# cnettel/cnF2freq

Measured on AMD Instinct MI355X. Metric: individual*marker fwd-bwd steps/sec (all 8 shift modes, forward+backward, dosage rows), higher is better.
Workload: dtype f64

## Files before the change

### cnf2freq_amd/csrc/cnf2_kernels.hip

```cpp
#include <hip/hip_runtime.h>

#include <string.h>
#include <type_traits>

#include "cnf2_device.h"
#include "cnf2_lane.h"
#include "cnf2_emtab.h"
#include "cnf2_accum.h"
#include "cnf2_acctab.h"
#include "cnf2_accpath.h"
#include "cnf2_variance.h"

namespace cnf2 {

template <int CTRL>
__device__ __forceinline__ double dpp_mov_all(double v)
{
    int lo = __builtin_amdgcn_mov_dpp(__double2loint(v), CTRL, 0xF, 0xF, true);
    int hi = __builtin_amdgcn_mov_dpp(__double2hiint(v), CTRL, 0xF, 0xF, true);
    return __hiloint2double(hi, lo);
}
template <int K>
__device__ __forceinline__ double swizzle_xor(double v)
{
// ... 884 lines not shown
struct RawSlots {
    uint8_t ap[4];
    double2 su[4];
    double  hw[4];
    double2 tq;
};

template <int TQ_SHIFT>
__device__ __forceinline__ void load_raw_at(const KernelParams& p, const FastCtx& c, int m, int lo_m, int hi_m, RawSlots* r)
{
    m = m < lo_m ? lo_m : (m > hi_m ? hi_m : m);
    const int32_t rows[4] = {c.row_root, c.row_par, c.row_tr, c.row_ot};
#pragma unroll
    for (int k = 0; k < 4; k++) {
        const size_t i = (size_t)rows[k] * p.n_markers + m;
        r->ap[k] = p.allele8[i];
        r->su[k] = p.sure[i];
        r->hw[k] = p.hw[i];
    }
    const int mt = m + TQ_SHIFT;
    r->tq        = p.tq[mt < 0 ? 0 : mt];
}
template <int TQ_SHIFT>
__device__ __forceinline__ void load_raw(const KernelParams& p, const FastCtx& c, int m0, int lo_m, int hi_m, RawSlots* r)
{
    load_raw_at<TQ_SHIFT>(p, c, m0 + c.mi, lo_m, hi_m, r);
}

template <bool CLASSES, bool HOMPAR = false, bool HOMLEAF = false, bool NORESTR = false, bool TIES = false, int STRIDE = TAB_STRIDE,
          int KOFF = 0>
__device__ __forceinline__ void produce_row(const FastCtx& c, double* tab, bool valid, const RawSlots& raw)
{
    if (valid) {
        const Slot root = unpack_slot(raw.ap[0], raw.su[0].x, raw.su[0].y, raw.hw[0]);
        const Slot par  = unpack_slot(raw.ap[1], raw.su[1].x, raw.su[1].y, raw.hw[1]);
        const Slot tr   = unpack_slot(raw.ap[2], raw.su[2].x, raw.su[2].y, raw.hw[2]);
        const Slot ot   = unpack_slot(raw.ap[3], raw.su[3].x, raw.su[3].y, raw.hw[3]);
        double  cw[2];
        double* row = tab + c.mi * STRIDE;
        double* rb = row + c.idx_base;
        emtab_part_to<CLASSES, HOMPAR, HOMLEAF, NORESTR, TIES>(c.pc, root, par, tr, ot,
                               [&](int kind, int e, double v) {
                                   if (KOFF > 0 && kind == 0) return;
                                   const int b  = e & 3;
                                   const int k  = b == 0 ? 0 : (b == 1 ? c.idx_k01 : (b == 2 ? c.idx_k10 : 6));
                                   rb[(kind == 0 ? 0 : (kind == 1 ? TAB_R : TAB_2) + KOFF) + (e >> 2) * 8 + k] = v;
                               },
                               cw);
        if (KOFF > 0) return;
        if ((c.part & 5) == 0) {
            row[TAB_C + c.pc.f * 2 + 0] = cw[0];
            row[TAB_C + c.pc.f * 2 + 1] = cw[1];
        }
        if (c.part == 0) *(double2*)(row + TAB_T) = raw.tq;
    }
}
template <bool CLASSES, bool TIES = false, int STRIDE = TAB_STRIDE, int KOFF = 0>
__device__ __forceinline__ void produce_tile(const KernelParams& p, const FastCtx& c, double* tab, int m0, int last,
                                             const RawSlots& raw, int hom)
{
    if (TIES) {
        produce_row<CLASSES, false, false, false, CLASSES, STRIDE, KOFF>(c, tab, m0 + c.mi <= last, raw);
        return;
    }
    if (hom == 2) produce_row<CLASSES, true, true, false, false, STRIDE>(c, tab, m0 + c.mi <= last, raw);
    else if (hom == 1) produce_row<CLASSES, true, false, false, false, STRIDE>(c, tab, m0 + c.mi <= last, raw);
    else if (hom == 3) produce_row<CLASSES, false, false, true, false, STRIDE>(c, tab, m0 + c.mi <= last, raw);
    else produce_row<CLASSES, false, false, false, false, STRIDE>(c, tab, m0 + c.mi <= last, raw);
}

struct RawRec {
    uint8_t  ap;
    double   s0, s1, hw;
    double   Bp, Cp, Kp, t0, t1, oo;
    uint32_t bits;
    double   tq0, tq1;
};
__device__ __forceinline__ int clamp_marker(int m, int lo_m, int hi_m) { return m < lo_m ? lo_m : (m > hi_m ? hi_m : m); }
__device__ __forceinline__ uint8_t load_root_allele(const KernelParams& p, const FastCtx& c, int m0, int lo_m, int hi_m)
{
    const __attribute__((address_space(1))) uint8_t* a8 = (const __attribute__((address_space(1))) uint8_t*)p.allele8;
    return a8[(size_t)c.row_root * p.n_markers + clamp_marker(m0 + c.mi, lo_m, hi_m)];
}
template <int TQ_SHIFT, bool ONE_MARKER = false>
__device__ __forceinline__ void load_rec(const KernelParams& p, const FastCtx& c, uint32_t rec_row, int m0, int lo_m, int hi_m,
                                         uint8_t ap, RawRec* r)
{
    const int     m = clamp_marker(m0 + c.mi, lo_m, hi_m);
    const size_t  i = (size_t)c.row_root * p.n_markers + m;
    const double2 su = p.sure[i];
    r->ap = ap;
    r->s0 = su.x;
    r->s1 = su.y;
    r->hw = p.hw[i];
    const int v = ((c.pc.P ^ c.pc.f) & 1) ? (ap >> 4) : (ap & 15);
    const double2* q = (const double2*)(p.line_rec + (((size_t)(rec_row + (uint32_t)m) * LINE_VALUES + v) * 2 + c.pc.firstpar));
    const double2 q0 = q[0], q1 = q[1], q2 = q[2];
    r->Bp   = q0.x;
    r->Cp   = q0.y;
    r->Kp   = q1.x;
    r->t0   = q1.y;
    r->t1   = q2.x;
    r->oo   = q2.y;
    r->bits = ((const uint32_t*)q)[12];
    const int mt = m + TQ_SHIFT;
    if (ONE_MARKER) {
        typedef double sd2 __attribute__((ext_vector_type(2)));
        const int mu = __builtin_amdgcn_readfirstlane(mt < 0 ? 0 : mt);
        const sd2 tq = ((const __attribute__((address_space(4))) sd2*)p.tq)[mu];
        r->tq0 = tq.x;
        r->tq1 = tq.y;
    } else {
        const double2 tq = p.tq[mt < 0 ? 0 : mt];
        r->tq0 = tq.x;
        r->tq1 = tq.y;
    }
}
template <bool CLASSES, bool PACKED = false>
__device__ __forceinline__ void produce_row_rec(const FastCtx& c, double* tab, bool valid, const RawRec& raw)
{
    if (valid) {
        const Slot root = unpack_slot(raw.ap, raw.s0, raw.s1, raw.hw);
        LineRec rec;
        rec.Bp   = raw.Bp;
        rec.Cp   = raw.Cp;
        rec.Kp   = raw.Kp;
        rec.t0   = raw.t0;
        rec.t1   = raw.t1;
        rec.oo   = raw.oo;
        rec.bits = raw.bits;
        double  cw[2];
        double* row = tab + c.mi * TAB_STRIDE;
        double* rb  = row + c.idx_base;
        emtab_part_rec<CLASSES, PACKED>(c.pc.P, c.pc.f, root, rec,
                                [&](int kind, int e, double v) {
                                    const int b = e & 3;
                                    const int k = b == 0 ? 0 : (b == 1 ? c.idx_k01 : (b == 2 ? c.idx_k10 : 6));
                                    rb[(kind == 0 ? 0 : (kind == 1 ? TAB_R : TAB_2)) + (e >> 2) * 8 + k] = v;
                                },
                                cw);
        if ((c.part & 5) == 0) {
            row[TAB_C + c.pc.f * 2 + 0] = cw[0];
            row[TAB_C + c.pc.f * 2 + 1] = cw[1];
        }
        if (c.part == 0) *(double2*)(row + TAB_T) = make_double2(raw.tq0, raw.tq1);
    }
}
__global__ __launch_bounds__(256) void line_records_kernel(const LineKey* lines, int n_lines, const uint8_t* allele8,
                                                           const double2* sure, const double* hw, int n_markers, LineRec* out)
{
    const size_t per_line = (size_t)n_markers * LINE_VALUES * 2;
    const size_t t        = (size_t)blockIdx.x * blockDim.x + threadIdx.x;
    if (t >= per_line * (size_t)n_lines) return;
    const int     firstpar = (int)(t & 1), v = (int)((t >> 1) & (LINE_VALUES - 1));
    const size_t  lm = t / (LINE_VALUES * 2);
    const int     m = (int)(lm % (size_t)n_markers);
    const LineKey k = lines[lm / (size_t)n_markers];
    auto slot = [&](int32_t row) {
        const size_t i = (size_t)row * n_markers + m;
        const double2 s = sure[i];
        return unpack_slot(allele8[i], s.x, s.y, hw[i]);
    };
    const Slot par = slot(k.row_par), ga = slot(k.row_a), gb = slot(k.row_b);
    LineRec r;
    line_record_make(k.fl_par, firstpar ? k.fl_b : k.fl_a, firstpar ? k.fl_a : k.fl_b, firstpar, v, par, firstpar ? gb : ga,
                     firstpar ? ga : gb, &r);
    out[t] = r;
}

struct RawOne {
    uint8_t ap;
    double2 su;
    double  hw;
    double2 tq;
};

template <int TQ_SHIFT>
// ... 1269 lines not shown
#pragma unroll
            for (int j = 0; j < NR; j++) S.b[j] *= e[j];
            const bool scale_here = !ODD && (ml & bmask) == 0;
            if (!ODD && __ballot(scale_here)) {
                double bb[NR] = {S.b[0], S.b[1]};
                double bm = S.bmant;
                int    be = S.bexpo;
                bool   bd = S.bdead;
                const double bsum = scale_chain<true>(bb, &bm, &be, &bd);
#pragma unroll
                for (int j = 0; j < NR; j++) S.b[j] = scale_here ? bb[j] : S.b[j];
                S.bmant = scale_here ? bm : S.bmant;
                S.bexpo = scale_here ? be : S.bexpo;
                S.bdead = scale_here ? bd : S.bdead;
                if (any_in_job(__ballot(scale_here && bsum > 0.0 && bsum * CNF2_RESCALE_GUARD < 1.0))) bmask = 1;
            }
            transition_uniform(S.b, r_m.x, r_m.y);
        };
        {
            const int mtop = first + (ntile - 1) * 2;
            load_rec<-1>(pq, cp, rec_row, mtop + moff, first, last, load_root_allele(pq, cp, mtop + moff, first, last), &rraw);
            ap_next = load_root_allele(pq, cp, mtop - 2 + moff, first, last);
        }
        const int    mi2 = lane >> 3, sub = lane & 7;
        for (int t = ntile - 1; t >= 0; t--) {
            const int m0 = first + t * 2;
            produce_row_rec<true, true>(cp, tab, m0 + pmt <= last, rraw);
            load_rec<-1>(pq, cp, rec_row, m0 - 2 + moff, first, last, ap_next, &rraw);
            ap_next = load_root_allele(pq, cp, m0 - 4 + moff, first, last);
            wave_lds_fence();
            if (m0 < last) {
                marker(odd_t(), myrow1, m0 + 1);
                marker(even_t(), myrow0, m0, true);
            } else marker(even_t(), myrow0, m0);
            wave_lds_fence();
            {
                const double* red = tab + mi2 * TS + sub * 8;
                double        d0 = 0.0, d1 = 0.0, d2 = 0.0;
#pragma unroll
                for (int i2 = 0; i2 < 8; i2++) {
                    d0 += red[i2];
                    d1 += red[64 + i2];
                    d2 += red[128 + i2];
                }
                d0 = chain_sum(d0);
                d1 = chain_sum(d1);
                d2 = chain_sum(d2);
                d0 = fmax(d0, 0.0);
                d1 = fmax(d1, 0.0);
                d2 = fmax(d2, 0.0);
                if (sub == 0 && m0 + (mi2 >> 2) <= last) {
                    if (!(p.flags & KP_RAW_DOSAGE)) {
                        const double tsum = d0 + d1 + d2;
                        const double inv  = tsum > 0.0 ? 1.0 / tsum : 0.0;
                        d0 *= inv;
                        d1 *= inv;
                        d2 *= inv;
                    }
                    int ei = eind;
                    asm volatile("" : "+v"(ei));
                    double* out = p.dosage + ((size_t)ei * p.n_markers + (m0 + (mi2 >> 2))) * 3;
                    out[0] = d0;
                    out[1] = d1;
                    out[2] = d2;
                }
            }
            wave_lds_fence();
        }
    }
    if (stamp && fresh_lane() == 0) {
        p.clock_out[0] = __builtin_readcyclecounter() - t_shader;
        p.clock_out[1] = wall_clock64() - t_wall;
    }
}

static_assert(TAB_R == 72 && TAB_2 == 136 && TAB_STRIDE >= 200, "up8_park (cnf2_lane.h) is written for this row layout");
static_assert(TAB_R % 2 == 0 && TAB_2 % 2 == 0 && TAB_STRIDE % 2 == 0, "the A-side runs of a chain (up8_sum_run) are read 16 bytes at a time");
#ifndef CNF2_UP8_ROW_SUMS
#define CNF2_UP8_ROW_SUMS 1
#endif
#ifndef CNF2_UP8_SCALAR_GAP
#define CNF2_UP8_SCALAR_GAP 1
#endif
#ifndef CNF2_UP8_FWD_TILE
#define CNF2_UP8_FWD_TILE 8
#endif
#ifndef CNF2_UP8_FWD_READ
#define CNF2_UP8_FWD_READ 2
#endif
static_assert(CNF2_UP8_FWD_TILE == 1 || (CNF2_UP8_FWD_TILE >= 2 && CNF2_UP8_FWD_TILE % 2 == 0), "a forward tile holds an even number of markers");
static_assert(CNF2_UP8_FWD_TILE == 1 || up8_fwd_buffers(CNF2_UP8_FWD_TILE, 8 * TAB_STRIDE) * CNF2_UP8_FWD_TILE * UP8_FWD_MARKER <= 8 * TAB_STRIDE,
              "the forward tiles live in the wave's eight table rows");
__device__ __forceinline__ void produce_slot_rec(const FastCtx& c, double* slot, const RawRec& raw)
{
    const Slot root = unpack_slot(raw.ap, raw.s0, raw.s1, raw.hw);
    LineRec rec;
    rec.Bp   = raw.Bp;
    rec.Cp   = raw.Cp;
    rec.Kp   = raw.Kp;
    rec.t0   = raw.t0;
    rec.t1   = raw.t1;
    rec.oo   = raw.oo;
    rec.bits = raw.bits;
    double  cw[2];
    double* d = slot + up8_fwd_at(0, c.mi, 0);
    emtab_part_rec<false, true>(c.pc.P, c.pc.f, root, rec,
                                [&](int, int e, double v) {
                                    if (e == 0) d[up8_fwd_at(0, 0, up8_fwd_part(c.part))] = v;
                                },
                                cw);
    if ((c.part & 5) == 0) {
        d[up8_fwd_at(0, 0, up8_fwd_weight(c.pc.f, 0))] = cw[0];
        d[up8_fwd_at(0, 0, up8_fwd_weight(c.pc.f, 1))] = cw[1];
    }
    if (c.part == 0) {
        d[up8_fwd_at(0, 0, up8_fwd_gap(0))] = raw.tq0;
        d[up8_fwd_at(0, 0, up8_fwd_gap(1))] = raw.tq1;
    }
}
struct Up8FwdRow {
    const double*  row;
    const FastCtx& c;
    __device__ __forceinline__ void emission(double (&e)[2], double k) const { emission_from_row(row, c, e, k); }
    __device__ __forceinline__ double2 gap() const { return *(const double2*)(row + TAB_T); }
};
struct Up8FwdSlot {
    double w0, a0, w1, a1, B0[2], B1[2], g0, g1;
    Up8FwdSlot() = default;
    __device__ __forceinline__ Up8FwdSlot(const double* a, const double* w, const double* b)
    {
        constexpr int F = up8_fwd_at(0, 0, 2);
        w0 = w[0];
        a0 = a[0];
        w1 = w[F];
        a1 = a[F];
#pragma unroll
        for (int j = 0; j < 2; j++) {
            B0[j] = b[up8_fwd_at(0, 0, j)];
            B1[j] = b[F + up8_fwd_at(0, 0, j)];
        }
        g0 = b[up8_fwd_at(0, 0, up8_fwd_gap(0) - 4)];
        g1 = b[up8_fwd_at(0, 0, up8_fwd_gap(1) - 4)];
    }
    __device__ __forceinline__ void emission(double (&e)[2], double k) const
    {
        const double cA0 = w0 * a0 * k;
        const double cA1 = w1 * a1 * k;
#pragma unroll
        for (int j = 0; j < 2; j++) e[j] = cA0 * B0[j] + cA1 * B1[j];
    }
    __device__ __forceinline__ double2 gap() const { return make_double2(g0, g1); }
};
__global__ __launch_bounds__(CNF2_BLOCK, CNF2_UNI_MIN_BLOCKS) void fb_unipack8_kernel(KernelParams p)
{
    constexpr int  NR = 2, ROW = UP8_SPILL_ROW, TS = TAB_STRIDE;
    constexpr bool SG = CNF2_UP8_SCALAR_GAP != 0;
    __shared__ __attribute__((aligned(16))) double lds[CNF2_WAVES_PER_BLOCK][8 * TS];

    const int wib   = __builtin_amdgcn_readfirstlane(threadIdx.x >> 6);
    const int wave  = blockIdx.x * CNF2_WAVES_PER_BLOCK + wib;
    const int nwave = gridDim.x * CNF2_WAVES_PER_BLOCK;
    double*   spill = p.spill + (size_t)wave * p.spill_stride;
    const bool stamp = p.clock_out != nullptr && wave == 0;
    unsigned long long t_shader = 0, t_wall = 0;
    if (stamp) {
        t_shader = __builtin_readcyclecounter();
        t_wall   = wall_clock64();
    }

    auto take_job = [&](int strided) {
        if (!p.job_next) return strided;
        int j = 0;
        if (fresh_lane() == 0) j = atomicAdd(p.job_next, 1);
        return __builtin_amdgcn_readfirstlane(j);
    };
    for (int job = take_job(wave); job < p.n_pjobs; job = take_job(job + nwave)) {
        const int        lane = fresh_lane();
        const PackedJob* pj   = p.pjobs + 2 * (size_t)job;
        int           wq   = wib;
        const Window* wins = p.windows;
        KernelParams  pq   = p;
        asm volatile("" : "+s"(wq), "+s"(wins), "+s"(pq.allele8));
        double* const tab = lds[wq];
        const int first = __builtin_amdgcn_readfirstlane(pj[0].first), last = __builtin_amdgcn_readfirstlane(pj[0].last);
        const int chrom = __builtin_amdgcn_readfirstlane(pj[0].chrom);
        FastCtx cp;
        cp.part = lane >> 3;
        cp.mi   = lane & 7;
        const int moff = -cp.mi;
        uint32_t  rec_row;
        {
            const int    pind = pj[cp.mi >> 2].ind[cp.mi & 3];
            const Window wp   = wins[pind];
            make_part(wp, cp.part, &cp.pc, &cp.row_par, &cp.row_tr, &cp.row_ot);
            cp.row_root = wp.row[0];
            rec_row     = (uint32_t)p.line_keys[2 * (size_t)pind + (cp.pc.P ? 1 : 0)] * (uint32_t)p.n_markers;
        }
        cp.idx_base = part_entry_index(cp.part, 0);
        cp.idx_k01  = part_entry_index(cp.part, 1) - cp.idx_base;
        cp.idx_k10  = part_entry_index(cp.part, 2) - cp.idx_base;
        const int rj = up8_job(lane), b0 = up8_b0(lane);
        const int ind = pj[rj >> 2].ind[rj & 3];
// ... 13 lines not shown
        auto any_in_job = [&](unsigned long long ballot) {
            unsigned tl = (unsigned)ballot, th = (unsigned)(ballot >> 32);
            tl |= tl >> 16;
            tl |= tl >> 8;
            th |= th >> 16;
            th |= th >> 8;
            return (((rj & 4) ? th : tl) & jbits) != 0;
        };
        double* const myrow = tab + rj * TS;
        const bool uspill = !(p.flags & KP_NO_DOSAGE);
        const int  uoff   = up8_spill_value(lane);
        const int  ioff   = up8_spill_inv(rj, c.s0);
        const bool vwr    = up8_spill_writer(lane) && uspill;
        const bool iwr    = b0 == 0 && vwr;

        using odd_t  = std::integral_constant<bool, true>;
        using even_t = std::integral_constant<bool, false>;

        double a[NR];
#pragma unroll
        for (int j = 0; j < NR; j++) a[j] = 1.0 / 64.0;
        double mant = 1.0;
        int    expo = 0;
        bool   dead = false;
        double pend = 1.0;
        int    rmask = CNF2_RESCALE_MASK, bmask = CNF2_RESCALE_MASK;
        auto fwd_step = [&](auto odd_tag, const auto& src, int m) {
            constexpr bool ODD = decltype(odd_tag)::value;
            double         e[NR];
            src.emission(e, pend);
            const double2 r  = src.gap();
            const int     ml = m - first;
            double*       sp = spill + (size_t)(ml >> 1) * ROW;
            if (!ODD) {
                double ep[NR];
                src.emission(ep, 1.0);
                const d2v v = {a[0], a[1]};
                const d2v w = {a[0] * ep[0], a[1] * ep[1]};
                if (vwr) {
                    __builtin_nontemporal_store(v, (d2v*)(sp + uoff));
                    __builtin_nontemporal_store(w, (d2v*)(sp + UP8_SPILL_EMIT + uoff));
                }
            }
#pragma unroll
            for (int j = 0; j < NR; j++) a[j] *= e[j];
            pend = 1.0;
            const bool norm_here = m == last || (!ODD && (ml & rmask) == 0);
            if (__ballot(norm_here)) {
                double       mt = mant;
                int          ex = expo;
                bool         dd = dead;
                const double inv = chain_normaliser<true>(a, &mt, &ex, &dd);
                mant = norm_here ? mt : mant;
                expo = norm_here ? ex : expo;
                dead = norm_here ? dd : dead;
                pend = norm_here ? inv : 1.0;
                if (any_in_job(__ballot(norm_here && inv > CNF2_RESCALE_GUARD))) rmask = 1;
                if (iwr && (!ODD || norm_here)) sp[ioff + (ODD ? 1 : 0)] = pend;
            } else if (!ODD) {
                if (iwr) sp[ioff] = 1.0;
            }
            if (m < last) transition_uniform(a, r.x, r.y);
        };
        RawRec  rraw;
        uint8_t ap_next;
        if constexpr (CNF2_UP8_FWD_TILE == 1) {
            const Up8FwdRow src{myrow, c};
            load_rec<0, SG>(pq, cp, rec_row, first + moff, first, last, load_root_allele(pq, cp, first + moff, first, last), &rraw);
            ap_next = load_root_allele(pq, cp, first + 1 + moff, first, last);
            for (int m = first; m <= last; m++) {
                produce_row_rec<false, true>(cp, tab, true, rraw);
                load_rec<0, SG>(pq, cp, rec_row, m + 1 + moff, first, last, ap_next, &rraw);
                ap_next = load_root_allele(pq, cp, m + 2 + moff, first, last);
                wave_lds_fence();
                if ((m - first) & 1) fwd_step(odd_t(), src, m);
                else fwd_step(even_t(), src, m);
                wave_lds_fence();
            }
        } else {
            constexpr int T = CNF2_UP8_FWD_TILE, REGION = 8 * TS;
            const double* const qa = tab + up8_fwd_at(0, rj, up8_fwd_part(b0));
            const double* const qc = tab + up8_fwd_at(0, rj, up8_fwd_weight(0, c.s0));
            const double* const qb = tab + up8_fwd_at(0, rj, up8_fwd_part(4));
            RawRec  rr[2];
            uint8_t ap[2];
            load_rec<0, SG>(pq, cp, rec_row, first + moff, first, last, load_root_allele(pq, cp, first + moff, first, last), &rr[0]);
            load_rec<0, SG>(pq, cp, rec_row, first + 1 + moff, first, last, load_root_allele(pq, cp, first + 1 + moff, first, last), &rr[1]);
            ap[0] = load_root_allele(pq, cp, first + 2 + moff, first, last);
            ap[1] = load_root_allele(pq, cp, first + 3 + moff, first, last);
            int tile = 0;
            for (int m0 = first; m0 <= last; m0 += T, tile++) {
                const int toff = up8_fwd_tile(T, REGION, tile);
#pragma unroll
                for (int t = 0; t < T; t++) {
                    produce_slot_rec(cp, tab + toff + up8_fwd_at(t, 0, 0), rr[t & 1]);
                    load_rec<0, SG>(pq, cp, rec_row, m0 + t + 2 + moff, first, last, ap[t & 1], &rr[t & 1]);
                    ap[t & 1] = load_root_allele(pq, cp, m0 + t + 4 + moff, first, last);
                }
                wave_lds_fence();
                auto slot_at = [&](int t) {
                    const int o = toff + up8_fwd_at(t, 0, 0);
                    return Up8FwdSlot(qa + o, qc + o, qb + o);
                };
                constexpr int RD = CNF2_UP8_FWD_READ < T ? CNF2_UP8_FWD_READ : T;
                static_assert(T % RD == 0, "a forward tile is read in equal parts");
#pragma unroll
                for (int t0 = 0; t0 < T; t0 += RD) {
                    Up8FwdSlot src[RD];
#pragma unroll
                    for (int t = 0; t < RD; t++) src[t] = slot_at(t0 + t);
#pragma unroll
                    for (int t = 0; t < RD; t++) {
                        if (t0 + t == 0 || m0 + t0 + t <= last) {
                            if ((t0 + t) & 1) fwd_step(odd_t(), src[t], m0 + t0 + t);
                            else fwd_step(even_t(), src[t], m0 + t0 + t);
                        }
                    }
                }
                if (up8_fwd_buffers(T, REGION) == 1) wave_lds_fence();
            }
            if (up8_fwd_buffers(T, REGION) == 2) wave_lds_fence();
        }

        const bool   alive  = !dead;
        const double emine  = alive ? (double)expo : -1e300;
        const double emaxd  = fmax(emine, lane_xor8(emine));
        const bool   any_alive = emaxd > -1e299;
        const int    emax   = any_alive ? (int)emaxd : 0;
        int          dsh    = expo - emax;
        dsh                 = dsh < -2000 ? -2000 : dsh;
        const double tmine  = alive ? ldexp(mant, dsh) : 0.0;
        double       T      = tmine + lane_xor8(tmine);
        T += T;
        T += T;
        if (b0 == 0 && c.s2 == 0) {
#pragma unroll
            for (int s1 = 0; s1 < 2; s1++) {
                const int s = c.s0 | (s1 << 1);
#pragma unroll
                for (int s2 = 0; s2 < 2; s2++) {
                    p.factors[je * 8 + (s | (s2 << 2))] = mant;
                    p.fexp[je * 8 + (s | (s2 << 2))]    = alive ? expo : CNF2_LEXP_DEAD;
                }
            }
        }
        if (jlead) {
            p.loglik[je] = any_alive ? T : 8.0;
            p.lexp[je]   = any_alive ? emax : CNF2_LEXP_DEAD;
        }
        if (p.flags & KP_NO_DOSAGE) continue;

        BwdState<NR> S;
#pragma unroll
        for (int j = 0; j < NR; j++) S.b[j] = 1.0;
        S.bmant = 1.0;
        S.bexpo = 0;
        S.bdead = false;
        S.fmant = mant;
        S.fexpo = expo;
        const double xm  = any_alive ? 1.0 / T : 0.0;
        const int    xe  = -emax;
        const bool   chain_on = alive && !(tmine * 2.3538526683701998e17 < T);
        double nx_am[NR], nx_inv_even, nx_inv_odd;
        auto ask_spill = [&](int mn) {
            const double* sp = spill + (size_t)(mn < 0 ? 0 : mn >> 1) * ROW;
            const d2v     v  = __builtin_nontemporal_load((const d2v*)(sp + ((mn & 1) ? UP8_SPILL_EMIT : 0) + uoff));
            nx_am[0]         = v.x;
            nx_am[1]         = v.y;
            const double2 iv = *(const double2*)(sp + ioff);
            nx_inv_even      = iv.x;
            nx_inv_odd       = iv.y;
        };
        auto take_spill = [&]() {
#pragma unroll
            for (int j = 0; j < NR; j++) S.am[j] = nx_am[j];
            S.inv_even = nx_inv_even;
            S.inv_odd  = nx_inv_odd;
        };
        ask_spill(last - first);

        auto marker = [&](auto odd_tag, double* row, int m) {
            constexpr bool ODD = decltype(odd_tag)::value;
// ... 102 lines not shown
                }
                int ei = ind;
                asm volatile("" : "+v"(ei));
                double* out = p.dosage + ((size_t)ei * p.n_markers + m) * 3;
                out[0] = d0;
                out[1] = d1;
                out[2] = d2;
            }
#else
#ifdef CNF2_X_NOPARK
            double x_sum[3];
#endif
#pragma unroll
            for (int h = 0; h < 2; h++) {
                const int s1 = 1 - h;
                double    q[4][3];
#pragma unroll
                for (int v = 0; v < 4; v++) {
                    double n_tot = 0.0, n_a1 = 0.0, n_b1 = 0.0, n_2 = 0.0;
#pragma unroll
                    for (int f = 0; f < 2; f++) {
                        const int    ia = (f << 4) | (s1 << 3) | b0 | (v << 1);
                        const double cf = f ? cf1 : cf0;
                        const double av = cf * row[TAB_R + ia], a1 = cf * row[TAB_2 + ia];
                        const double sb = z[2 * f], sb1 = z[2 * f + 1];
                        n_tot += av * sb;
                        n_a1 += a1 * sb;
                        n_b1 += av * sb1;
                        n_2 += a1 * sb1;
                    }
                    q[v][2] = scale * n_2;
                    q[v][1] = scale * (n_a1 + n_b1 - 2.0 * n_2);
                    q[v][0] = scale * (n_tot - n_a1 - n_b1 + n_2);
#ifdef CNF2_X_NOPARK
#pragma unroll
                    for (int k = 0; k < 3; k++) x_sum[k] = (h == 0 && v == 0 ? 0.0 : x_sum[k]) + q[v][k];
#endif
                }
#ifndef CNF2_X_NOPARK
                wave_lds_fence();
#pragma unroll
                for (int v = 0; v < 4; v++) {
                    const int vl = up8_virtual_lane(lane, s1, v);
                    row[up8_park(0, vl)] = q[v][0];
                    row[up8_park(1, vl)] = q[v][1];
                    row[up8_park(2, vl)] = q[v][2];
                }
#endif
            }
#ifdef CNF2_X_NOPARK
            {
                const double d0 = fmax(chain_sum(x_sum[0]), 0.0), d1 = fmax(chain_sum(x_sum[1]), 0.0), d2 = fmax(chain_sum(x_sum[2]), 0.0);
                const double tsum = d0 + d1 + d2;
                const double inv  = (p.flags & KP_RAW_DOSAGE) ? 1.0 : (tsum > 0.0 ? 1.0 / tsum : 0.0);
                if ((lane & 7) == 0) {
                    int ei = eind;
                    asm volatile("" : "+v"(ei));
                    double* out = p.dosage + ((size_t)ei * p.n_markers + m) * 3;
                    out[0] = d0 * inv;
                    out[1] = d1 * inv;
                    out[2] = d2 * inv;
                }
            }
#endif
#endif
#pragma unroll
            for (int j = 0; j < NR; j++) S.b[j] *= e[j];
            const bool scale_here = !ODD && (ml & bmask) == 0;
            if (!ODD && __ballot(scale_here)) {
                double bb[NR] = {S.b[0], S.b[1]};
                double bm = S.bmant;
                int    be = S.bexpo;
                bool   bd = S.bdead;
                const double bsum = scale_chain<true>(bb, &bm, &be, &bd);
#pragma unroll
                for (int j = 0; j < NR; j++) S.b[j] = scale_here ? bb[j] : S.b[j];
                S.bmant = scale_here ? bm : S.bmant;
                S.bexpo = scale_here ? be : S.bexpo;
                S.bdead = scale_here ? bd : S.bdead;
                if (any_in_job(__ballot(scale_here && bsum > 0.0 && bsum * CNF2_RESCALE_GUARD < 1.0))) bmask = 1;
            }
            transition_uniform(S.b, r_m.x, r_m.y);
        };
        load_rec<-1, SG>(pq, cp, rec_row, last + moff, first, last, load_root_allele(pq, cp, last + moff, first, last), &rraw);
        ap_next = load_root_allele(pq, cp, last - 1 + moff, first, last);
#if !CNF2_UP8_ROW_SUMS && !defined(CNF2_X_NOPARK)
        const int mi2 = lane >> 3, sub = lane & 7;
#endif
        for (int m = last; m >= first; m--) {
            take_spill();
            ask_spill(m - first - 1);
            produce_row_rec<true, true>(cp, tab, true, rraw);
            load_rec<-1, SG>(pq, cp, rec_row, m - 1 + moff, first, last, ap_next, &rraw);
            ap_next = load_root_allele(pq, cp, m - 2 + moff, first, last);
            wave_lds_fence();
            if ((m - first) & 1) marker(odd_t(), myrow, m);
            else marker(even_t(), myrow, m);
#if !CNF2_UP8_ROW_SUMS && !defined(CNF2_X_NOPARK)
            wave_lds_fence();
            {
                const double *red0 =tab + mi2 * TS + up8_park(0, sub * 8), *red1 = tab + mi2 * TS + up8_park(1, sub * 8),
                             *red2 = tab + mi2 * TS + up8_park(2, sub * 8);
                double        d0 = 0.0, d1 = 0.0, d2 = 0.0;
#pragma unroll
                for (int i2 = 0; i2 < 8; i2++) {
                    d0 += red0[i2];
                    d1 += red1[i2];
                    d2 += red2[i2];
                }
                d0 = chain_sum(d0);
                d1 = chain_sum(d1);
                d2 = chain_sum(d2);
                d0 = fmax(d0, 0.0);
                d1 = fmax(d1, 0.0);
                d2 = fmax(d2, 0.0);
                if (sub == 0) {
                    if (!(p.flags & KP_RAW_DOSAGE)) {
                        const double tsum = d0 + d1 + d2;
                        const double inv  = tsum > 0.0 ? 1.0 / tsum : 0.0;
                        d0 *= inv;
                        d1 *= inv;
                        d2 *= inv;
                    }
                    int ei = eind;
                    asm volatile("" : "+v"(ei));
                    double* out = p.dosage + ((size_t)ei * p.n_markers + m) * 3;
                    out[0] = d0;
                    out[1] = d1;
                    out[2] = d2;
                }
            }
#endif
            wave_lds_fence();
        }
    }
    if (stamp && fresh_lane() == 0) {
        p.clock_out[0] = __builtin_readcyclecounter() - t_shader;
        p.clock_out[1] = wall_clock64() - t_wall;
    }
}

__global__ __launch_bounds__(256) void likelihood_logs_kernel(KernelParams p)
{
    const int t = blockIdx.x * blockDim.x + threadIdx.x;
    if (t >= p.n_jobs * 8) return;
    const Job    jb   = p.jobs[t >> 3];
    const int    s    = t & 7;
    const size_t e    = (size_t)jb.ind * p.n_chrom + jb.chrom;
    const double logk = p.chrom_logk[jb.chrom];
    const double ln2  = 0.69314718055994530942;
    const int    fe   = p.fexp[e * 8 + s];
    double       fs;
    if (fe == CNF2_LEXP_IGNORED) fs = CNF2_IGNORED_D;
    else if (fe == CNF2_LEXP_DEAD) fs = (double)CNF2_MINFACTOR_F;
    else fs = log(p.factors[e * 8 + s]) + (double)fe * ln2 + logk;
    p.factors[e * 8 + s] = fs;
    if (s == 0) {
        const int    le = p.lexp[e];
        const double T  = p.loglik[e];
        p.loglik[e] = (le == CNF2_LEXP_DEAD) ? (double)CNF2_MINFACTOR_F + log(T) : log(T) + (double)le * ln2 + logk;
    }
}
static void launch_likelihood_logs(const KernelParams& p, hipStream_t stream)
{
    if (p.n_jobs > 0) hipLaunchKernelGGL(likelihood_logs_kernel, dim3((p.n_jobs * 8 + 255) / 256), dim3(256), 0, stream, p);
}

__global__ __launch_bounds__(256) void loo_finish_kernel(double* loo, double* unl, int n_ind, int n_markers, double* loo_sum,
                                                         double* unl_sum)
{
    const int m = blockIdx.x * blockDim.x + threadIdx.x;
    if (m >= n_markers) return;
    double sl = 0.0, su = 0.0;
    for (int i = 0; i < n_ind; i++) {
        const size_t o = (size_t)i * n_markers + m;
        const double r = loo[o], u = unl[o];
        const bool   skipped = r < 0.0;
        const double lr = skipped ? CNF2_IGNORED_D : log(r), lu = skipped ? CNF2_IGNORED_D : -log(u);
// ... 3006 lines not shown
```

### cnf2freq_amd/csrc/cnf2_lane.h

```cpp
#ifndef CNF2_LANE_H
#define CNF2_LANE_H

#include "cnf2_emission.h"
#include "cnf2_window.h"

namespace cnf2 {

struct LaneJob {
    LineCfg cfg;
    int32_t row_par, row_tr, row_ot;
    int8_t  tie_par, tie_tr, tie_ot;
    int     P, f;
};

CNF2_HD void make_lane(const Window& w, int lane, LaneJob* L)
{
    const int P = lane >> 5, f = (lane >> 4) & 1, sp = (lane >> 3) & 1, k = lane & 7;
    const int firstpar = k & 1, upflag = k >> 1;
    const int slot_par = 1 + 3 * P;
    const int slot_tr  = slot_par + 1 + firstpar;
    const int slot_ot  = slot_par + 1 + (firstpar ^ 1);
    L->P = P;
    L->f = f;
    L->cfg.par      = w.flags[slot_par];
    L->cfg.tr       = w.flags[slot_tr];
    L->cfg.ot       = w.flags[slot_ot];
    L->cfg.firstpar = firstpar;
    L->cfg.bit_tr   = (upflag >> firstpar) & 1;
    L->cfg.bit_ot   = (upflag >> (firstpar ^ 1)) & 1;
    L->cfg.sp       = sp;
    L->row_par = w.row[slot_par] < 0 ? 0 : w.row[slot_par];
    L->row_tr  = w.row[slot_tr] < 0 ? 0 : w.row[slot_tr];
    L->row_ot  = w.row[slot_ot] < 0 ? 0 : w.row[slot_ot];
    L->tie_par = w.tie[slot_par];
    L->tie_tr  = w.tie[slot_tr];
    L->tie_ot  = w.tie[slot_ot];
}

CNF2_HD constexpr int state_lo(int lane) { return (lane & 7) ^ ((lane & 4) ? 3 : 0); }

enum { UNI_SPILL_INV = 32, UNI_SPILL_ROW = 48 };
CNF2_HD bool uni_spill_writer(int lane) { return (state_lo(lane) & 6) == 0; }
CNF2_HD int uni_spill_value(int lane) { return (lane >> 3) * 4 + (state_lo(lane) & 1) * 2; }
CNF2_HD int uni_spill_inv(int chain) { return UNI_SPILL_INV + 2 * chain; }

CNF2_HD int upk_job(int lane) { return (state_lo(lane) >> 1) & 3; }
CNF2_HD int upk_virtual_lane(int lane, int v) { return (lane & ~7) | state_lo((state_lo(lane) & 1) | (v << 1)); }
enum { UPK_SPILL_INV = 128, UPK_SPILL_ROW = 192 };
CNF2_HD int upk_spill_value(int lane) { return 2 * lane; }
CNF2_HD int upk_spill_inv(int job, int chain) { return UPK_SPILL_INV + 2 * (8 * job + chain); }

CNF2_HD int up8_job(int lane) { return ((lane >> 3) & 4) | ((state_lo(lane) >> 1) & 3); }
CNF2_HD int up8_s0(int lane) { return (lane >> 3) & 1; }
CNF2_HD int up8_s2(int lane) { return (lane >> 4) & 1; }
CNF2_HD int up8_b0(int lane) { return state_lo(lane) & 1; }
CNF2_HD int up8_virtual_lane(int lane, int s1, int v)
{
    return (up8_s0(lane) | (s1 << 1) | (up8_s2(lane) << 2)) * 8 + state_lo(up8_b0(lane) | (v << 1));
}
CNF2_HD int up8_sum_s1(int lane) { return up8_b0(lane); }
CNF2_HD constexpr int up8_place_b(int i2) { return state_lo(i2) & 1; }
CNF2_HD constexpr int up8_place_v(int i2) { return state_lo(i2) >> 1; }
CNF2_HD constexpr int up8_partner(int lane, int level) { return lane ^ (level == 0 ? 8 : (level == 1 ? 1 : 16)); }
CNF2_HD int up8_sum_run(int f, int s1) { return (f << 4) | (s1 << 3); }
CNF2_HD int up8_park(int cls, int vl)
{
    const int s = vl >> 3, s1 = (s >> 1) & 1, i4 = (s & 1) | ((s >> 2) << 1);
    const int base = s1 ? (cls == 0 ? 0 : (cls == 1 ? 32 : 104)) : (cls == 0 ? 72 : (cls == 1 ? 136 : 168));
    return base + i4 * 8 + (vl & 7);
}
enum { UP8_SPILL_EMIT = 64, UP8_SPILL_INV = 128, UP8_SPILL_ROW = 160 };
CNF2_HD bool up8_spill_writer(int lane) { return up8_s2(lane) == 0; }
CNF2_HD int up8_spill_value(int lane) { return 2 * (((lane >> 5) << 4) | (lane & 15)); }
CNF2_HD int up8_spill_emit(int lane) { return UP8_SPILL_EMIT + up8_spill_value(lane); }
CNF2_HD int up8_spill_inv(int job, int s0) { return UP8_SPILL_INV + 2 * (2 * job + s0); }

enum { UP8_FWD_SLOT = 16, UP8_FWD_VALUES = 14, UP8_FWD_MARKER = 8 * UP8_FWD_SLOT };
CNF2_HD constexpr int up8_fwd_buffers(int T, int region) { return 2 * T * UP8_FWD_MARKER <= region ? 2 : 1; }
CNF2_HD constexpr int up8_fwd_tile(int T, int region, int tile) { return up8_fwd_buffers(T, region) == 2 ? (tile & 1) * T * UP8_FWD_MARKER : 0; }
CNF2_HD constexpr int up8_fwd_at(int t, int job, int i) { return (t * UP8_FWD_SLOT + i) * 8 + job; }
CNF2_HD constexpr int up8_fwd_part(int part) { return part; }
CNF2_HD constexpr int up8_fwd_weight(int f, int s0) { return 8 + 2 * f + s0; }
CNF2_HD constexpr int up8_fwd_gap(int k) { return 12 + k; }

CNF2_HD int tie_force(int8_t tie, int combo)
{
    return tie < 0 ? -1 : ((combo >> tie) & 1);
}

CNF2_HD Slot unpack_slot(uint8_t allele_pair, double s0, double s1, double hw)
{
    Slot d;
    d.a0 = allele_pair & 15;
    d.a1 = allele_pair >> 4;
    d.s0 = s0;
    d.s1 = s1;
    d.hw = hw;
    return d;
}

}
#endif
```

Before: 5.951 billion.

## Stage per-marker root data through LDS in forward and backward up8 loops

Adds a staging scheme in which each lane loads the root allele, sure pair and hw value for a marker a tile ahead, writes them into spare LDS in the wave's table rows, and the per-marker loop then reads them back from LDS. This replaces the per-marker scattered global loads (and the serial allele-then-record dependency) in both the forward tile loop and the backward marker loop with cooperative prefetches. It is double-buffered and on by default. In exchange it uses more LDS space and adds LDS traffic and index arithmetic. An ablation path that loads root data once per tile, off by default, is also added.

```diff
diff --git a/cnf2freq_amd/csrc/cnf2_kernels.hip b/cnf2freq_amd/csrc/cnf2_kernels.hip
--- a/cnf2freq_amd/csrc/cnf2_kernels.hip
+++ b/cnf2freq_amd/csrc/cnf2_kernels.hip
@@ -990,17 +990,44 @@
     const __attribute__((address_space(1))) uint8_t* a8 = (const __attribute__((address_space(1))) uint8_t*)p.allele8;
     return a8[(size_t)c.row_root * p.n_markers + clamp_marker(m0 + c.mi, lo_m, hi_m)];
 }
-template <int TQ_SHIFT, bool ONE_MARKER = false>
-__device__ __forceinline__ void load_rec(const KernelParams& p, const FastCtx& c, uint32_t rec_row, int m0, int lo_m, int hi_m,
-                                         uint8_t ap, RawRec* r)
-{
-    const int     m = clamp_marker(m0 + c.mi, lo_m, hi_m);
-    const size_t  i = (size_t)c.row_root * p.n_markers + m;
+#ifndef CNF2_X_ROOTONCE
+#define CNF2_X_ROOTONCE 0
+#endif
+#if CNF2_X_ROOTONCE
+struct RawRoot {
+    uint8_t ap;
+    double  s0, s1, hw;
+    __device__ __forceinline__ void into(RawRec* r) const
+    {
+        r->ap = ap;
+        r->s0 = s0;
+        r->s1 = s1;
+        r->hw = hw;
+    }
+};
+__device__ __forceinline__ void load_root(const KernelParams& p, const FastCtx& c, int m0, int lo_m, int hi_m, RawRoot* r)
+{
+    const size_t  i  = (size_t)c.row_root * p.n_markers + clamp_marker(m0 + c.mi, lo_m, hi_m);
     const double2 su = p.sure[i];
-    r->ap = ap;
+    r->ap = load_root_allele(p, c, m0, lo_m, hi_m);
     r->s0 = su.x;
     r->s1 = su.y;
     r->hw = p.hw[i];
+}
+#endif
+template <int TQ_SHIFT, bool ONE_MARKER = false, bool ROOT = true>
+__device__ __forceinline__ void load_rec(const KernelParams& p, const FastCtx& c, uint32_t rec_row, int m0, int lo_m, int hi_m,
+                                         uint8_t ap, RawRec* r)
+{
+    const int     m = clamp_marker(m0 + c.mi, lo_m, hi_m);
+    r->ap = ap;
+    if (ROOT) {
+        const size_t  i = (size_t)c.row_root * p.n_markers + m;
+        const double2 su = p.sure[i];
+        r->s0 = su.x;
+        r->s1 = su.y;
+        r->hw = p.hw[i];
+    }
     const int v = ((c.pc.P ^ c.pc.f) & 1) ? (ap >> 4) : (ap & 15);
     const double2* q = (const double2*)(p.line_rec + (((size_t)(rec_row + (uint32_t)m) * LINE_VALUES + v) * 2 + c.pc.firstpar));
     const double2 q0 = q[0], q1 = q[1], q2 = q[2];
@@ -2436,6 +2463,15 @@
 #ifndef CNF2_UP8_SCALAR_GAP
 #define CNF2_UP8_SCALAR_GAP 1
 #endif
+#ifndef CNF2_UP8_ROOT_STAGE
+#define CNF2_UP8_ROOT_STAGE 1
+#endif
+#ifndef CNF2_UP8_ROOT_STAGE_FWD
+#define CNF2_UP8_ROOT_STAGE_FWD CNF2_UP8_ROOT_STAGE
+#endif
+#ifndef CNF2_UP8_ROOT_STAGE_BWD
+#define CNF2_UP8_ROOT_STAGE_BWD CNF2_UP8_ROOT_STAGE
+#endif
 #ifndef CNF2_UP8_FWD_TILE
 #define CNF2_UP8_FWD_TILE 8
 #endif
@@ -2472,6 +2508,34 @@
         d[up8_fwd_at(0, 0, up8_fwd_gap(1))] = raw.tq1;
     }
 }
+struct StagedRoot {
+    double2  su;
+    double   hw;
+    uint32_t ap;
+};
+__device__ __forceinline__ void load_stage(const KernelParams& p, const FastCtx& c, int m, int lo_m, int hi_m, StagedRoot* s)
+{
+    const __attribute__((address_space(1))) uint8_t* a8 = (const __attribute__((address_space(1))) uint8_t*)p.allele8;
+    const size_t i = (size_t)c.row_root * p.n_markers + clamp_marker(m, lo_m, hi_m);
+    s->su = p.sure[i];
+    s->hw = p.hw[i];
+    s->ap = a8[i];
+}
+__device__ __forceinline__ void store_stage_fwd(double* e, const StagedRoot& s)
+{
+    *(double2*)(e + UP8_STAGE_SURE)    = s.su;
+    e[UP8_STAGE_HW]                    = s.hw;
+    *(uint32_t*)(e + UP8_STAGE_ALLELE) = s.ap;
+}
+__device__ __forceinline__ void store_stage_bwd(double* row, int buf, int t, const StagedRoot& s)
+{
+    *(double2*)(row + (buf ? up8_stage_bwd_sure(1, 0) : up8_stage_bwd_sure(0, 0)) + 8 * t) = s.su;
+    row[(buf ? up8_stage_bwd_hw(1, 0) : up8_stage_bwd_hw(0, 0)) + 8 * t]                   = s.hw;
+    ((uint8_t*)(row + up8_stage_bwd_alleles(0) + buf))[t]                                  = (uint8_t)s.ap;
+}
+static_assert(up8_stage_bwd_sure(0, 3) == up8_stage_bwd_sure(0, 0) + 24 && up8_stage_bwd_hw(1, 3) == up8_stage_bwd_hw(1, 0) + 24 &&
+              up8_stage_bwd_alleles(1) == up8_stage_bwd_alleles(0) + 1, "store_stage_bwd and the staged readers step by marker and by buffer");
+static_assert(up8_stage_bwd_alleles(1) < TAB_R && up8_stage_bwd_alleles(0) >= TAB_T + 2, "the allele bytes sit behind the gap's factors");
 struct Up8FwdRow {
     const double*  row;
     const FastCtx& c;
@@ -2651,22 +2715,83 @@
             const double* const qa = tab + up8_fwd_at(0, rj, up8_fwd_part(b0));
             const double* const qc = tab + up8_fwd_at(0, rj, up8_fwd_weight(0, c.s0));
             const double* const qb = tab + up8_fwd_at(0, rj, up8_fwd_part(4));
-            RawRec  rr[2];
-            uint8_t ap[2];
-            load_rec<0, SG>(pq, cp, rec_row, first + moff, first, last, load_root_allele(pq, cp, first + moff, first, last), &rr[0]);
-            load_rec<0, SG>(pq, cp, rec_row, first + 1 + moff, first, last, load_root_allele(pq, cp, first + 1 + moff, first, last), &rr[1]);
-            ap[0] = load_root_allele(pq, cp, first + 2 + moff, first, last);
-            ap[1] = load_root_allele(pq, cp, first + 3 + moff, first, last);
+            constexpr bool STAGE = CNF2_UP8_ROOT_STAGE_FWD != 0 && T == UP8_STAGE_T && up8_fwd_buffers(T, REGION) == 1 &&
+                                   up8_stage_fwd_room(T, REGION) >= 2 * UP8_STAGE_BUFFER;
+            constexpr int SB = UP8_STAGE_BUFFER, SM = 8 * UP8_STAGE_ENTRY;
+            double* const       sgw = tab + up8_stage_fwd_at(T, REGION, 0, cp.part, cp.mi);
+            const double* const sgr = tab + up8_stage_fwd_at(T, REGION, 0, 0, cp.mi);
+            auto allele_at = [&](const double* e) { return (uint8_t) * (const uint32_t*)(e + UP8_STAGE_ALLELE); };
+            StagedRoot sg;
+            RawRec     rr[2];
+            uint8_t    ap[2];
+            if constexpr (STAGE) {
+                StagedRoot sg1;
+                load_stage(pq, cp, first + cp.part, first, last, &sg);
+                load_stage(pq, cp, first + T + cp.part, first, last, &sg1);
+                store_stage_fwd(sgw, sg);
+                store_stage_fwd(sgw + SB, sg1);
+                load_stage(pq, cp, first + 2 * T + cp.part, first, last, &sg);
+                wave_lds_fence();
+                load_rec<0, SG, false>(pq, cp, rec_row, first + moff, first, last, allele_at(sgr), &rr[0]);
+                load_rec<0, SG, false>(pq, cp, rec_row, first + 1 + moff, first, last, allele_at(sgr + SM), &rr[1]);
+                ap[0] = allele_at(sgr + 2 * SM);
+                ap[1] = allele_at(sgr + 3 * SM);
+            } else {
+                load_rec<0, SG>(pq, cp, rec_row, first + moff, first, last, load_root_allele(pq, cp, first + moff, first, last), &rr[0]);
+                load_rec<0, SG>(pq, cp, rec_row, first + 1 + moff, first, last, load_root_allele(pq, cp, first + 1 + moff, first, last), &rr[1]);
+                ap[0] = load_root_allele(pq, cp, first + 2 + moff, first, last);
+                ap[1] = load_root_allele(pq, cp, first + 3 + moff, first, last);
+            }
+#if CNF2_X_ROOTONCE & 1
+            static_assert(!STAGE, "the ablation is of the per-marker loads");
+            RawRoot rt_cur, rt_nxt;
+            load_root(pq, cp, first + moff, first, last, &rt_cur);
+            load_root(pq, cp, first + T + moff, first, last, &rt_nxt);
+#endif
             int tile = 0;
             for (int m0 = first; m0 <= last; m0 += T, tile++) {
                 const int toff = up8_fwd_tile(T, REGION, tile);
-#pragma unroll
-                for (int t = 0; t < T; t++) {
-                    produce_slot_rec(cp, tab + toff + up8_fwd_at(t, 0, 0), rr[t & 1]);
-                    load_rec<0, SG>(pq, cp, rec_row, m0 + t + 2 + moff, first, last, ap[t & 1], &rr[t & 1]);
-                    ap[t & 1] = load_root_allele(pq, cp, m0 + t + 4 + moff, first, last);
-                }
+                if constexpr (STAGE) {
+                    const double* const cur = sgr + (tile & 1) * SB;
+                    const double* const nxt = sgr + ((tile & 1) ^ 1) * SB;
+                    double2 su = *(const double2*)(cur + UP8_STAGE_SURE);
+                    double  hw = cur[UP8_STAGE_HW];
+#pragma unroll
+                    for (int t = 0; t < T; t++) {
+                        rr[t & 1].s0 = su.x;
+                        rr[t & 1].s1 = su.y;
+                        rr[t & 1].hw = hw;
+                        if (t + 1 < T) {
+                            su = *(const double2*)(cur + (t + 1) * SM + UP8_STAGE_SURE);
+                            hw = cur[(t + 1) * SM + UP8_STAGE_HW];
+                        }
+                        produce_slot_rec(cp, tab + toff + up8_fwd_at(t, 0, 0), rr[t & 1]);
+                        load_rec<0, SG, false>(pq, cp, rec_row, m0 + t + 2 + moff, first, last, ap[t & 1], &rr[t & 1]);
+                        ap[t & 1] = allele_at(t + 4 < T ? cur + (t + 4) * SM : nxt + (t + 4 - T) * SM);
+                    }
+                } else {
+#pragma unroll
+                    for (int t = 0; t < T; t++) {
+#if CNF2_X_ROOTONCE & 1
+                        rt_cur.into(&rr[t & 1]);
+                        produce_slot_rec(cp, tab + toff + up8_fwd_at(t, 0, 0), rr[t & 1]);
+                        load_rec<0, SG, false>(pq, cp, rec_row, m0 + t + 2 + moff, first, last, rt_cur.ap, &rr[t & 1]);
+#else
+                        produce_slot_rec(cp, tab + toff + up8_fwd_at(t, 0, 0), rr[t & 1]);
+                        load_rec<0, SG>(pq, cp, rec_row, m0 + t + 2 + moff, first, last, ap[t & 1], &rr[t & 1]);
+                        ap[t & 1] = load_root_allele(pq, cp, m0 + t + 4 + moff, first, last);
+#endif
+                    }
+                }
+#if CNF2_X_ROOTONCE & 1
+                rt_cur = rt_nxt;
+                load_root(pq, cp, m0 + 2 * T + moff, first, last, &rt_nxt);
+#endif
                 wave_lds_fence();
+                if constexpr (STAGE) {
+                    store_stage_fwd(sgw + (tile & 1) * SB, sg);
+                    load_stage(pq, cp, m0 + 3 * T + cp.part, first, last, &sg);
+                }
                 auto slot_at = [&](int t) {
                     const int o = toff + up8_fwd_at(t, 0, 0);
                     return Up8FwdSlot(qa + o, qc + o, qb + o);
@@ -2935,18 +3060,73 @@
             }
             transition_uniform(S.b, r_m.x, r_m.y);
         };
-        load_rec<-1, SG>(pq, cp, rec_row, last + moff, first, last, load_root_allele(pq, cp, last + moff, first, last), &rraw);
-        ap_next = load_root_allele(pq, cp, last - 1 + moff, first, last);
+        constexpr bool STAGE_B = CNF2_UP8_ROOT_STAGE_BWD != 0 && CNF2_UP8_ROW_SUMS != 0;
+        double* const prow = tab + cp.mi * TS;
+        auto staged_sure = [&](int d) {
+            return *(const double2*)(prow + (((d >> 3) & 1) ? up8_stage_bwd_sure(1, 0) : up8_stage_bwd_sure(0, 0)) + 8 * (d & 7));
+        };
+        auto staged_hw = [&](int d) { return prow[(((d >> 3) & 1) ? up8_stage_bwd_hw(1, 0) : up8_stage_bwd_hw(0, 0)) + 8 * (d & 7)]; };
+        auto staged_allele = [&](int d) { return ((const uint8_t*)(prow + up8_stage_bwd_alleles(0) + ((d >> 3) & 1)))[d & 7]; };
+        StagedRoot sgb;
+        double2    su_n;
+        double     hw_n;
+        if constexpr (STAGE_B) {
+            load_stage(pq, cp, last - cp.part, first, last, &sgb);
+            store_stage_bwd(prow, 0, cp.part, sgb);
+            load_stage(pq, cp, last - 8 - cp.part, first, last, &sgb);
+            wave_lds_fence();
+            load_rec<-1, SG, false>(pq, cp, rec_row, last + moff, first, last, staged_allele(0), &rraw);
+            ap_next = staged_allele(1);
+            su_n    = staged_sure(0);
+            hw_n    = staged_hw(0);
+        } else {
+            load_rec<-1, SG>(pq, cp, rec_row, last + moff, first, last, load_root_allele(pq, cp, last + moff, first, last), &rraw);
+            ap_next = load_root_allele(pq, cp, last - 1 + moff, first, last);
+        }
+#if CNF2_X_ROOTONCE & 2
+        static_assert(!STAGE_B, "the ablation is of the per-marker loads");
+        RawRoot rt_cur, rt_nxt;
+        load_root(pq, cp, last + moff, first, last, &rt_cur);
+        load_root(pq, cp, last - 8 + moff, first, last, &rt_nxt);
+#endif
 #if !CNF2_UP8_ROW_SUMS && !defined(CNF2_X_NOPARK)
         const int mi2 = lane >> 3, sub = lane & 7;
 #endif
         for (int m = last; m >= first; m--) {
             take_spill();
             ask_spill(m - first - 1);
+#if CNF2_X_ROOTONCE & 2
+            rt_cur.into(&rraw);
             produce_row_rec<true, true>(cp, tab, true, rraw);
-            load_rec<-1, SG>(pq, cp, rec_row, m - 1 + moff, first, last, ap_next, &rraw);
-            ap_next = load_root_allele(pq, cp, m - 2 + moff, first, last);
+            load_rec<-1, SG, false>(pq, cp, rec_row, m - 1 + moff, first, last, rt_cur.ap, &rraw);
+            if (((last - m) & 7) == 7) {
+                rt_cur = rt_nxt;
+                load_root(pq, cp, m - 9 + moff, first, last, &rt_nxt);
+            }
+#else
+            if constexpr (STAGE_B) {
+                const int d = last - m;
+                rraw.s0 = su_n.x;
+                rraw.s1 = su_n.y;
+                rraw.hw = hw_n;
+                produce_row_rec<true, true>(cp, tab, true, rraw);
+                load_rec<-1, SG, false>(pq, cp, rec_row, m - 1 + moff, first, last, ap_next, &rraw);
+                ap_next = staged_allele(d + 2);
+                su_n    = staged_sure(d + 1);
+                hw_n    = staged_hw(d + 1);
+            } else {
+                produce_row_rec<true, true>(cp, tab, true, rraw);
+                load_rec<-1, SG>(pq, cp, rec_row, m - 1 + moff, first, last, ap_next, &rraw);
+                ap_next = load_root_allele(pq, cp, m - 2 + moff, first, last);
+            }
+#endif
             wave_lds_fence();
+            if constexpr (STAGE_B) {
+                if (((last - m) & 7) == 0) {
+                    store_stage_bwd(prow, (((last - m) >> 3) + 1) & 1, cp.part, sgb);
+                    load_stage(pq, cp, m - 16 - cp.part, first, last, &sgb);
+                }
+            }
             if ((m - first) & 1) marker(odd_t(), myrow, m);
             else marker(even_t(), myrow, m);
 #if !CNF2_UP8_ROW_SUMS && !defined(CNF2_X_NOPARK)
diff --git a/cnf2freq_amd/csrc/cnf2_lane.h b/cnf2freq_amd/csrc/cnf2_lane.h
--- a/cnf2freq_amd/csrc/cnf2_lane.h
+++ b/cnf2freq_amd/csrc/cnf2_lane.h
@@ -83,6 +83,17 @@
 CNF2_HD constexpr int up8_fwd_weight(int f, int s0) { return 8 + 2 * f + s0; }
 CNF2_HD constexpr int up8_fwd_gap(int k) { return 12 + k; }
 
+enum { UP8_STAGE_T = 8, UP8_STAGE_ENTRY = 4, UP8_STAGE_BUFFER = UP8_STAGE_T * 8 * UP8_STAGE_ENTRY };
+CNF2_HD constexpr int up8_stage_fwd_room(int T, int region) { return region - up8_fwd_buffers(T, region) * T * UP8_FWD_MARKER; }
+CNF2_HD constexpr int up8_stage_fwd_at(int T, int region, int buf, int t, int job)
+{
+    return up8_fwd_buffers(T, region) * T * UP8_FWD_MARKER + buf * UP8_STAGE_BUFFER + (t * 8 + job) * UP8_STAGE_ENTRY;
+}
+enum { UP8_STAGE_SURE = 0, UP8_STAGE_HW = 2, UP8_STAGE_ALLELE = 3 };
+CNF2_HD constexpr int up8_stage_bwd_sure(int buf, int t) { return 8 * t + (buf ? 6 : 2); }
+CNF2_HD constexpr int up8_stage_bwd_hw(int buf, int t) { return 8 * t + (buf ? 5 : 4); }
+CNF2_HD constexpr int up8_stage_bwd_alleles(int buf) { return 70 + buf; }
+
 CNF2_HD int tie_force(int8_t tie, int combo)
 {
     return tie < 0 ? -1 : ((combo >> tie) & 1);
```

After: 6.528 billion, median of 6. +9.7%, better.
